# HazyResearch/flash-fft-conv

Measured on AMD Instinct MI355X. Metric: FFT-conv fwd+bwd seq/s, B=16 H=768 L=16384 fft=32768 bf16, higher is better.
Workload: dtype bf16; 1 GPU; FlashFFTConv(32768) B=16 H=768 L=16384 bf16, fwd+bwd incl. k->k_f and dk (BASELINE configs[1]); heads_per_rank=768, parallelism=head-shard x1 (no collective)

## Files before the change

flash-fft-conv_amd/csrc/ffc_body.h:

```cpp
#pragma once
#include <stdint.h>

#include "ffc_layout.h"
#include "ffc_plan.h"

#ifndef FFC_FN
#define FFC_FN inline __attribute__((always_inline))
#endif

namespace ffc {

struct ConvArgs {
  const void* u;
  const void* pregate;
  const void* postgate;
  void* y;
  const void* kf;
  const uint8_t* tab;
  PlanTabs t;
  int B, H, L;
  int npair;
  int nchunk, ppc;
  int conj_kf;
  int fast;
  float s_inv;
  float s_fwd;
  int flags;
  int stream;
  int persist;
  int R;
  int64_t sbu, sbg, sbp, sby;
  void* zsave;
  void* yraw;
  int sparse;
  unsigned long long* prof;
  const void* aux_in;
  void* aux_out;
  int64_t sbai, sbao;
  const float* kfuse_k;
  const void* kfuse_x;
  int kfuse_Lk, kfuse_fast;
  float kfuse_scale;
  const void* addend;
  int64_t sba;
};

struct Pass {
  int k0 = 0, R = 1;
  const uint8_t* mat_fwd = nullptr;
  const uint8_t* mat_inv = nullptr;
};

template <class B, class GEO, int DT>
struct Body {
  using f32 = typename B::f32;
  using i32 = typename B::i32;
  using u32 = typename B::u32;
  using pred = typename B::pred;
  using U2 = typename B::U2;
  using U4 = typename B::U4;
  using A16 = typename B::A16;
  using W4 = typename B::W4;

  struct Mat { W4 w[2][3]; };
  struct CT16 { A16 re, im; };
  struct Op { W4 r[2], i[2]; };

  static FFC_FN void load_mat(Mat& m, const uint8_t* p, i32 lane) {
#pragma unroll
// ... 1570 lines not shown
    }
  }
  static FFC_FN void z_load(const void* zs, int tau, KfRegs& z, bool nt = false) {
    const i32 lane = B::opaque(B::lane());
    const i32 c = lane & 31, hi = lane >> 5;
    if (nt) {
#pragma unroll
      for (int rq = 0; rq < 4; rq++) z.v[rq] = B::g_r128_nt(zs, ((hi + (tau * 8 + 2 * rq)) * 32 + c));
      return;
    }
#pragma unroll
    for (int rq = 0; rq < 4; rq++) z.v[rq] = B::g_r128(zs, ((hi + (tau * 8 + 2 * rq)) * 32 + c));
  }
  static FFC_FN uint8_t* z_slot(void* base, int h, int npair, int p) {
    return (uint8_t*)base + ((int64_t)h * npair + p) * ((int64_t)GEO::N * 4);
  }
  static FFC_FN uint8_t* z_slot_small(void* base, int h, int npair, int q, int R, int k0) {
    const int ntile = (npair + GEO::G - 1) / GEO::G;
    return (uint8_t*)base + (((int64_t)h * ntile + q) * R + k0) * 4096;
  }
  static FFC_FN uint8_t* z_slot_rp(void* base, int h, int npair, int p, int R, int k0) {
    return (uint8_t*)base + (((int64_t)h * npair + p) * R + k0) * ((int64_t)GEO::N * 4);
  }
  static FFC_FN void load_kf(const ConvArgs& a, int h, int tau, KfRegs& k) {
    const i32 lane = B::opaque(B::lane());
    const i32 c = lane & 31, hi = lane >> 5;
    const uint8_t* kfh = (const uint8_t*)a.kf + (int64_t)h * (GEO::NT * 1024 * 4);
    if (a.flags & 2) {
#pragma unroll
      for (int rq = 0; rq < 4; rq++) k.v[rq] = B::g_r128_nt(kfh, ((hi + (tau * 8 + 2 * rq)) * 32 + c));
      return;
    }
#pragma unroll
    for (int rq = 0; rq < 4; rq++) k.v[rq] = B::g_r128(kfh, ((hi + (tau * 8 + 2 * rq)) * 32 + c));
  }
  template <bool IP = false, bool SZ = false>
  static FFC_FN void inner_tile(const ConvArgs& a, int tau, const InnerRegs& R, Unit un, const KfRegs& kf, const InnerPass* ip = nullptr,
                                uint8_t* zs = nullptr) {
    A16 re, im;
    tile_fwd<true, IP>(tau, R, un, re, im, ip);
    if constexpr (SZ) {
      if (GEO::OUTER || zs) z_store(zs, 0, re, im, Z_STREAM);
    }
#pragma unroll
    for (int rq = 0; rq < 4; rq++) {
      u32 wv[4] = {kf.v[rq].x, kf.v[rq].y, kf.v[rq].z, kf.v[rq].w};
#pragma unroll
      for (int q = 0; q < 4; q++) {
        f32 kr = B::template unpack_lo<DT>(wv[q]), ki = B::template unpack_hi<DT>(wv[q]);
        if (a.conj_kf) ki = B::fconst(0.f) - ki;
// ... 726 lines not shown
```

flash-fft-conv_amd/csrc/ffc_k_bwd.hip:

```cpp
#include "ffc_bwd_launch.h"

template <int DT>
__global__ __launch_bounds__(256) void mul_rows_kernel(const uint16_t* __restrict__ x, const uint16_t* __restrict__ y, uint16_t* __restrict__ out,
                                                       int64_t HL, int64_t sbx, int64_t sby, int64_t sbo, int fast) {
  const int b = blockIdx.y;
  const uint16_t* xb = x + b * sbx; const uint16_t* yb = y + b * sby; uint16_t* ob = out + b * sbo;
  if (fast) {
    for (int64_t i = (int64_t)blockIdx.x * blockDim.x + threadIdx.x; i < HL / 8; i += (int64_t)gridDim.x * blockDim.x) {
      const u32x4v a = __builtin_nontemporal_load((const u32x4v*)xb + i), c = __builtin_nontemporal_load((const u32x4v*)yb + i);
      u32x4v o;
#pragma unroll
      for (int q = 0; q < 4; q++)
        o[q] = DevB::pack<DT>(DevB::unpack_lo<DT>(a[q]) * DevB::unpack_lo<DT>(c[q]), DevB::unpack_hi<DT>(a[q]) * DevB::unpack_hi<DT>(c[q]));
      __builtin_nontemporal_store(o, (u32x4v*)ob + i);
    }
  } else {
    for (int64_t i = (int64_t)blockIdx.x * blockDim.x + threadIdx.x; i < HL; i += (int64_t)gridDim.x * blockDim.x)
      ob[i] = (uint16_t)DevB::pack<DT>(DevB::unpack_lo<DT>(xb[i]) * DevB::unpack_lo<DT>(yb[i]), 0.f);
  }
}


extern "C" int ffc_conv_bwd(const ffc_plan* p, const void* dout, const void* u, const void* kf, const void* pregate,
                            const void* postgate, void* du, void* dpre, void* ws, int64_t B, int64_t H, int64_t L, void* stream) {
  return ffc_conv_bwd_gated(p, dout, u, kf, pregate, postgate, du, dpre, nullptr, ws, B, H, L, stream);
}
struct BwdCall {
  const void *dout, *u, *kf, *pregate, *postgate;
  void *du, *dpre, *dpost, *ws;
  int64_t B, H, L;
  void* stream;
  int64_t sb_dout, sb_u, sb_pre, sb_post, sb_du, sb_dpre, sb_dpost;
  const void *zin, *yraw;
  float* dk; int64_t Lk;
  void* dk_pair; float dk_pair_scale;
  bool* dk_done;
};
static BwdCall bwd_call(const void* dout, const void* u, const void* kf, const void* pregate, const void* postgate, void* du, void* dpre,
                        void* dpost, void* ws, int64_t B, int64_t H, int64_t L, void* stream) {
  BwdCall c{};
  c.dout = dout; c.u = u; c.kf = kf; c.pregate = pregate; c.postgate = postgate; c.du = du; c.dpre = dpre; c.dpost = dpost; c.ws = ws;
  c.B = B; c.H = H; c.L = L; c.stream = stream;
  return c;
}
static void bwd_strides(BwdCall* c, int64_t sb_dout, int64_t sb_u, int64_t sb_pre, int64_t sb_post, int64_t sb_du, int64_t sb_dpre, int64_t sb_dpost) {
  c->sb_dout = sb_dout; c->sb_u = sb_u; c->sb_pre = sb_pre; c->sb_post = sb_post; c->sb_du = sb_du; c->sb_dpre = sb_dpre; c->sb_dpost = sb_dpost;
}
static int conv_bwd_impl(const ffc_plan* p, const BwdCall& c) {
  const void *dout = c.dout, *u = c.u, *kf = c.kf, *pregate = c.pregate, *postgate = c.postgate, *zin = c.zin, *yraw = c.yraw;
  void *du = c.du, *dpre = c.dpre, *dpost = c.dpost, *ws = c.ws, *stream = c.stream;
  const int64_t B = c.B, H = c.H, L = c.L, Lk = c.Lk;
  int64_t sb_dout = c.sb_dout, sb_u = c.sb_u, sb_pre = c.sb_pre, sb_post = c.sb_post, sb_du = c.sb_du, sb_dpre = c.sb_dpre, sb_dpost = c.sb_dpost;
  if (!p || !dout || !kf || !du || !ws) return ffc_fail("null arg");
  if (!u && (!zin || pregate || postgate || dpre || (dpost && !yraw))) return ffc_fail("null u: only with saved spectra and no gates");
  if (yraw && !dpost) return ffc_fail("y_raw needs a dpost output");
  if (yraw && !zin && p->hp.N1 > 1) return ffc_fail("y_raw without the saved spectra: single-tile sizes (fft <= 2048) only");
  if (zin && (ffc_spectrum_bytes(p, B, H) == 0 || ((uintptr_t)zin & 15))) return ffc_fail("spectrum buffer: unsupported plan or misaligned");
  if (B <= 0 || H <= 0) return ffc_fail("empty batch/heads");
  if (L <= 0 || L > p->hp.N) return ffc_fail("L must be in (0, fft_size]");
// ... 27 lines not shown
  if (c.dk_pair && c.dk_done && !((uintptr_t)c.dk_pair & 15) && bwd_dk_form(p->hp, a.nchunk, p->env_flags, true) != DK_SEPARATE) {
    set_dk_tail(&d, nullptr, c.dk_pair, p->hp.N, c.dk_pair_scale, 1, p->d_blob_bf, p->hp_bf.tabs);
    *c.dk_done = true;
  }
  d.dpost = (p->hp.N1 > 1 || yraw) ? dpost : nullptr;
  d.zin = zin;
  d.yraw = yraw;
  if (yraw && p->hp.R > 1 && p->hp.N1 > 1) {
    const int64_t HL = H * L;
    const int fast = (HL % 8 == 0) && !((sb_dout | sb_dpost) & 7) && !(((uintptr_t)dout | (uintptr_t)yraw | (uintptr_t)dpost) & 15);
    int64_t nb = (HL / (fast ? 8 : 1) + 255) / 256;
    if (nb > 8192) nb = 8192;
    const dim3 grid((unsigned)nb, (unsigned)B), block(256);
    if (p->hp.dtype == DT_BF16)
      hipLaunchKernelGGL(mul_rows_kernel<DT_BF16>, grid, block, 0, (hipStream_t)stream, (const uint16_t*)dout, (const uint16_t*)yraw,
                         (uint16_t*)dpost, HL, sb_dout, HL, sb_dpost, fast);
    else
      hipLaunchKernelGGL(mul_rows_kernel<DT_F16>, grid, block, 0, (hipStream_t)stream, (const uint16_t*)dout, (const uint16_t*)yraw,
                         (uint16_t*)dpost, HL, sb_dout, HL, sb_dpost, fast);
    HIPCHK(hipGetLastError());
    d.dpost = nullptr; d.yraw = nullptr; dpost = nullptr;
  }
  if (d.dpost && ((((uintptr_t)dpost) | (uintptr_t)yraw) & 15)) a.fast = 0;
  int rc = (zin && p->hp.N1 > 1) ? ffc_bwdz_launch(p->hp.N, p->hp.dtype, d, (hipStream_t)stream)
                                 : ffc_dispatch<BwdLaunchZ<0>::T>(p->hp.N, p->hp.dtype, d, (hipStream_t)stream);
  if (rc || !dpost || d.dpost) return rc;
  return ffc_conv_fwd_strided(p, u, kf, pregate, dout, dpost, B, H, L, 0, sb_u, sb_pre, sb_dout, sb_dpost, stream);
}
extern "C" int ffc_conv_bwd_gated_strided(const ffc_plan* p, const void* dout, const void* u, const void* kf, const void* pregate,
                                          const void* postgate, void* du, void* dpre, void* dpost, void* ws, int64_t B, int64_t H,
                                          int64_t L, int64_t sb_dout, int64_t sb_u, int64_t sb_pre, int64_t sb_post,
                                          int64_t sb_du, int64_t sb_dpre, int64_t sb_dpost, void* stream) {
  BwdCall c = bwd_call(dout, u, kf, pregate, postgate, du, dpre, dpost, ws, B, H, L, stream);
  bwd_strides(&c, sb_dout, sb_u, sb_pre, sb_post, sb_du, sb_dpre, sb_dpost);
  return conv_bwd_impl(p, c);
}
extern "C" int ffc_conv_bwd_z(const ffc_plan* p, const void* dout, const void* u, const void* kf, const void* pregate,
                              const void* postgate, void* du, void* dpre, void* dpost, void* ws, const void* zin, int64_t B, int64_t H,
                              int64_t L, int64_t sb_dout, int64_t sb_u, int64_t sb_pre, int64_t sb_post,
                              int64_t sb_du, int64_t sb_dpre, int64_t sb_dpost, void* stream) {
  if (!zin) return ffc_fail("null spectrum buffer");
  BwdCall c = bwd_call(dout, u, kf, pregate, postgate, du, dpre, dpost, ws, B, H, L, stream);
  bwd_strides(&c, sb_dout, sb_u, sb_pre, sb_post, sb_du, sb_dpre, sb_dpost);
  c.zin = zin;
  return conv_bwd_impl(p, c);
}
// ... 1 lines not shown
                               const void* postgate, void* du, void* dpre, void* dpost, void* ws, const void* zin, const void* y_raw,
                               int64_t B, int64_t H, int64_t L, int64_t sb_dout, int64_t sb_u, int64_t sb_pre, int64_t sb_post,
                               int64_t sb_du, int64_t sb_dpre, int64_t sb_dpost, void* stream) {
  if ((!zin && !(p && p->hp.N1 <= 1)) || !y_raw || !dpost) return ffc_fail("null spectrum / y_raw / dpost buffer (y_raw alone: single-tile sizes, fft <= 2048)");
  BwdCall c = bwd_call(dout, u, kf, pregate, postgate, du, dpre, dpost, ws, B, H, L, stream);
  bwd_strides(&c, sb_dout, sb_u, sb_pre, sb_post, sb_du, sb_dpre, sb_dpost);
  c.zin = zin; c.yraw = y_raw;
  return conv_bwd_impl(p, c);
}
extern "C" int ffc_conv_bwd_gated(const ffc_plan* p, const void* dout, const void* u, const void* kf, const void* pregate,
                                  const void* postgate, void* du, void* dpre, void* dpost, void* ws, int64_t B, int64_t H,
                                  int64_t L, void* stream) {
  return ffc_conv_bwd_gated_strided(p, dout, u, kf, pregate, postgate, du, dpre, dpost, ws, B, H, L, 0, 0, 0, 0, 0, 0, 0, stream);
}

extern "C" int ffc_conv_bwd_k(const ffc_plan* p, const void* dout, const void* u, const void* kf, const void* pregate, const void* postgate,
                              void* du, void* dpre, void* dpost, void* ws, const void* zin, const void* y_raw, float* dk, int64_t Lk,
                              int64_t B, int64_t H, int64_t L, void* stream) {
  if (!dk) return ffc_fail("null dk");
  bool dk_done = false;
  BwdCall c = bwd_call(dout, u, kf, pregate, postgate, du, dpre, dpost, ws, B, H, L, stream);
  c.zin = zin; c.yraw = ((zin || p->hp.N1 <= 1) && y_raw && dpost) ? y_raw : nullptr;
  c.dk = dk; c.Lk = Lk; c.dk_done = &dk_done;
  int rc = conv_bwd_impl(p, c);
  if (rc || dk_done) return rc;
  return ffc_kernel_ifft_grad(p, ws, B, H, Lk, dk, stream);
}

extern "C" int ffc_conv_bwd_kx(const ffc_plan* p, const void* dout, const void* u, const void* kf, void* du, void* ws, const void* zin,
                               void* outpair, float scale, int64_t B, int64_t H, int64_t L, void* stream) {
  if (!outpair) return ffc_fail("null outpair");
  bool dk_done = false;
  BwdCall c = bwd_call(dout, u, kf, nullptr, nullptr, du, nullptr, nullptr, ws, B, H, L, stream);
  c.zin = zin; c.dk_pair = outpair; c.dk_pair_scale = scale; c.dk_done = &dk_done;
  int rc = conv_bwd_impl(p, c);
  if (rc || dk_done) return rc;
  return ffc_kernel_ifft_grad_c(p, ws, B, H, outpair, scale, stream);
}
```

flash-fft-conv_amd/csrc/ffc_modes.h:

```cpp
#pragma once
#include "ffc_body.h"

namespace ffc {

struct KfArgs {
  const float* k;
  void* kf;
  const uint8_t* tab;
  PlanTabs t;
  int H, Lk;
  float scale;
  float s_fwd;
  float prescale;
  const void* xpair;
  int fast;
  int R;
};

struct DkfArgs {
  ConvArgs c;
  const void* dout;
  float* ws;
  int64_t sbd, sbdu, sbdpre, sbdpost;
  void* du;
// ... 175 lines not shown
#pragma unroll
      for (int q = 0; q < 4; q++) w[q] = B::template pack<DT>(re[4 * rq + q] * a.scale, im[4 * rq + q] * a.scale);
      v.x = w[0]; v.y = w[1]; v.z = w[2]; v.w = w[3];
      if constexpr (GEO::OUTER) {
        pred ok = (c * 0 + unit_id) < a.H * hmul;
        i32 idx = ((hi + (tau * 8 + 2 * rq)) * 32 + c) + unit_id * (GEO::NT * 256);
        B::g_w128(a.kf, idx, v, ok);
      } else {
        i32 V = hi * 4 + 8 * rq;
        i32 sV = V / GEO::N3, k3 = V % GEO::N3, sU = c / GEO::N2, k2 = c % GEO::N2;
        i32 hd = sU * GEO::SV + sV + unit_id * GEO::G;
        pred ok = hd < a.H;
#pragma unroll
        for (int su = 0; su < GEO::SU; su++)
#pragma unroll
          for (int sv = 0; sv < GEO::SV; sv++) {
            i32 rho = (k3 + sv * GEO::N3) >> 2;
            i32 idx = (rho * 32 + (k2 + su * GEO::N2)) + hd * 256;
            B::g_w128(a.kf, idx, v, ok);
          }
      }
    }
  }
  static FFC_FN void kf_store_flat(const KfArgs& a, int hrow, const A16& re, const A16& im, int hlim) {
    const i32 lane = B::opaque(B::lane());
    const i32 c = lane & 31, hi = lane >> 5;
#pragma unroll
    for (int rq = 0; rq < 4; rq++) {
      U4 v;
      v.x = B::template pack<DT>(re[4 * rq] * a.scale, im[4 * rq] * a.scale);
      v.y = B::template pack<DT>(re[4 * rq + 1] * a.scale, im[4 * rq + 1] * a.scale);
      v.z = B::template pack<DT>(re[4 * rq + 2] * a.scale, im[4 * rq + 2] * a.scale);
      v.w = B::template pack<DT>(re[4 * rq + 3] * a.scale, im[4 * rq + 3] * a.scale);
      B::g_w128(a.kf, ((hi + 2 * rq) * 32 + c) + hrow * 256, v, (c * 0 + hrow) < hlim);
    }
  }
  static FFC_FN void kfft(const KfArgs& a, int wg) {
    BD::setup_tables(a.tab, a.t);
    const int wv = B::wave();
    Unit un;
    un.wq = wv % GEO::NW;
    const int u = wv / GEO::NW;
    un.eb = u * GEO::EBYTES;
    const int unit_id = wg * GEO::UPW + u;
    const int nunits = GEO::OUTER ? a.H : (a.H + GEO::G - 1) / GEO::G;
    const bool act = unit_id < nunits;
// ... 24 lines not shown
              kf_store(a, unit_id * a.R + k0, un.wq * GEO::TPW + tt, re, im, a.R);
            }
          }
          B::barrier();
        }
        return;
      }
    }
    if constexpr (GEO::OUTER) {
      if (act) {
        if (a.xpair) {
          ConvArgs cv{};
          cv.u = a.xpair; cv.B = 2; cv.H = a.H; cv.L = GEO::N; cv.fast = 1; cv.sbu = (int64_t)a.H * GEO::N;
          BD::rows_in(cv, unit_id, 0, un);
        } else {
          k_rows_in(a, unit_id, un);
        }
        B::lds_fence();
        if ((GEO::N1 / 2) * GEO::Mi >= a.Lk) BD::template outer_stage<true, true>(a.Lk, un, a.s_fwd);
        else BD::template outer_stage<true, false>(a.Lk, un, a.s_fwd);
      }
      B::barrier();
      if (act) {
#pragma unroll 1
        for (int tt = 0; tt < GEO::TPW; tt++) {
          A16 re, im;
          BD::tile_fwd(un.wq * GEO::TPW + tt, R, un, re, im);
          kf_store(a, unit_id, un.wq * GEO::TPW + tt, re, im);
        }
      }
    } else if (a.R > 1) {
      if constexpr (GEO::N == 1024) {
        BD::setup_tables_ipass(a.tab, a.t, a.R);
        if (act) {
#pragma unroll 1
          for (int k0 = 0; k0 < a.R; k0++) {
            Pass ps; ps.k0 = k0; ps.R = a.R;
            InnerPass ip;
            BD::load_inner_pass(ip, k0);
            k_rows_in_rp(a, unit_id, un, ps);
            B::lds_fence();
            A16 re, im;
            BD::template tile_fwd<true, true, false, true>(0, R, un, re, im, &ip);
            kf_store_flat(a, unit_id * a.R + k0, re, im, a.H * a.R);
            B::lds_fence();
          }
        }
      }
    } else {
      if (act) {
        k_rows_in(a, unit_id, un);
// ... 12 lines not shown
    a.k = c.kfuse_k; a.kf = const_cast<void*>(c.kf); a.H = c.H; a.Lk = c.kfuse_Lk; a.scale = c.kfuse_scale; a.s_fwd = c.s_fwd;
    a.prescale = DT == DT_F16 ? 256.f : 1.f;
    a.fast = c.kfuse_fast;
    Unit un;
    un.wq = B::wave() % GEO::NW;
    un.eb = 0;
    if (unit == 0) {
      if (c.kfuse_x) {
        ConvArgs cv{};
        cv.u = c.kfuse_x; cv.B = 2; cv.H = c.H; cv.L = GEO::N; cv.fast = 1; cv.sbu = (int64_t)c.H * GEO::N;
        BD::rows_in(cv, h, 0, un);
        a.Lk = GEO::N; a.prescale = 1.0f;
      } else {
        k_rows_in(a, h, un);
      }
      B::lds_fence();
      if ((GEO::N1 / 2) * GEO::Mi >= a.Lk) BD::template outer_stage<true, true>(a.Lk, un, a.s_fwd);
      else BD::template outer_stage<true, false>(a.Lk, un, a.s_fwd);
    }
    B::barrier();
    if (unit == 0) {
      InnerRegs R;
      BD::load_inner(R, un);
#pragma unroll 1
      for (int tt = 0; tt < GEO::TPW; tt++) {
        A16 re, im;
        BD::tile_fwd(un.wq * GEO::TPW + tt, R, un, re, im);
        kf_store(a, h, un.wq * GEO::TPW + tt, re, im);
      }
    }
    B::barrier();
  }

  struct ZReg { u32 r[8], i[8]; };
  static FFC_FN void z_pack(const A16& re, const A16& im, ZReg& z) {
#pragma unroll
    for (int q = 0; q < 8; q++) {
      z.r[q] = B::template pack<DT>(re[2 * q], re[2 * q + 1]);
      z.i[q] = B::template pack<DT>(im[2 * q], im[2 * q + 1]);
    }
  }
  using BD::z_store;
  using BD::z_load;
  static FFC_FN void w_accum_z(float* slab, int tau, bool first, const typename BD::KfRegs& zv, const A16& re, const A16& im) {
    const i32 lane = B::opaque(B::lane());
    const i32 c = lane & 31, hi = lane >> 5;
#pragma unroll
    for (int rq = 0; rq < 4; rq++) {
      i32 idx = ((hi + (tau * 8 + 2 * rq)) * 32 + c) * 2;
      u32 wv[4] = {zv.v[rq].x, zv.v[rq].y, zv.v[rq].z, zv.v[rq].w};
      f32 wr[4], wi[4];
// ... 248 lines not shown
        }
        re[r] = sr * d.dk_scale; im[r] = si * d.dk_scale;
      }
      BD::template tile_inv<false>(d.c.s_inv, un.wq * GEO::TPW + T, R, un, re, im);
    }
    B::barrier();
  }
  static FFC_FN void dk_tail_multi(const DkfArgs& d, int h, int u, int wq) {
    static_assert(GEO::UPW > 1 && GEO::TPW == 4, "dk tail: sums in registers");
    const Unit un = unit_of(u, wq);
    const i32 lane = B::opaque(B::lane());
    B::barrier();
    InnerRegs R;
    if (u == 0) BD::template load_inner<false>(R, un);
    dk_tail_tile_multi<0>(d, u, un, R, lane); dk_tail_tile_multi<1>(d, u, un, R, lane);
    dk_tail_tile_multi<2>(d, u, un, R, lane); dk_tail_tile_multi<3>(d, u, un, R, lane);
    if (u == 0) {
      BD::template outer_stage<false, false>(d.Lk, un);
      B::lds_fence();
      dk_tail_rows(d, h, un);
    }
    B::barrier();
  }
  template <bool WITH_DX, bool RP = false, bool ZSAVED = false>
  static FFC_FN void bwd_tiles(const ConvArgs& a, int h, Unit un, const InnerRegs& R, const void* zs, float* slab, bool first, WAcc& W,
                               Pass ps = Pass(), bool z_stream = false, bool second = false) {
    static_assert(GEO::TPW == 4, "one accumulator block a[32 T ..] per tile slot of the wave");
    constexpr bool FOLD = BD::CAN_FOLD && GEO::N1 == 32 && WITH_DX && !RP && ZSAVED;
    const uint8_t* fold = FOLD ? a.tab + a.t.fold : nullptr;
    typename BD::KfRegs zv;
    typename BD::Mat2 fa;
    if constexpr (FOLD) BD::load_mat2_issue(fa, fold + (un.wq * GEO::TPW) * 6144, B::opaque(B::lane()));
#pragma unroll 1
    for (int tt = 0; tt < GEO::TPW; tt++) {
      const int tau = un.wq * GEO::TPW + tt;
      if constexpr (WITH_DX && GEO::NW > 1) {
        if (tt == GEO::TPW / 2) { if (second) B::template setprio<2>(); else B::template setprio<1>(); }
      }
      z_load(zs, tau, zv, z_stream || (a.flags & 4) != 0);
      typename BD::KfRegs kf;
      constexpr bool KFL = FOLD;
      if constexpr (WITH_DX && !KFL) BD::load_kf(a, h, tau, kf);
      A16 re, im;
      BD::template tile_fwd<false, false, FOLD>(tau, R, un, re, im, nullptr, fold, FOLD ? &fa : nullptr);
      if constexpr (WITH_DX && KFL) BD::load_kf(a, h, tau, kf);
      switch (tt) {
        case 0: w_acc_tile<0>(zv, re, im); break;
        case 1: w_acc_tile<1>(zv, re, im); break;
        case 2: w_acc_tile<2>(zv, re, im); break;
        default: w_acc_tile<3>(zv, re, im); break;
      }
      if constexpr (WITH_DX) {
        typename BD::Mat2 g[2];
        if constexpr (FOLD) {
          const i32 lane = B::opaque(B::lane());
          BD::load_mat2_issue(g[0], fold + (2 * GEO::NT + tau) * 6144, lane);
          BD::load_mat2_issue(g[1], fold + (3 * GEO::NT + tau) * 6144, lane);
        }
        kf_conj_mul(kf, re, im);
        if constexpr (FOLD) {
          const int tn = tt + 1 < GEO::TPW ? tau + 1 : tau;
          BD::load_mat2_issue(fa, fold + tn * 6144, B::opaque(B::lane()));
        }
        BD::template tile_inv<false, RP, false, FOLD>(a.s_inv, tau, R, un, re, im, 0, ps, nullptr, fold, FOLD ? g : nullptr);
      }
    }
  }
  template <bool HALF = false, bool RP = false>
  static FFC_FN void dkf(const DkfArgs& d, int h, int chunk, int wg_linear, int k0 = 0, int wv_in = 0) {
    const ConvArgs& a = d.c;
    const Pass ps = RP ? make_pass(a.tab, a.t, a.R, k0) : Pass();
    constexpr int NCX = HALF ? BD::NCH / 2 : BD::NCH;
    if constexpr (!RP) BD::setup_tables(a.tab, a.t);
    const int wv = RP ? wv_in : B::wave();
    Unit un;
    un.wq = wv % GEO::NW;
    const int u = wv / GEO::NW;
    un.eb = u * GEO::EBYTES;
    const int p0 = chunk * a.ppc;
    int p1 = p0 + a.ppc;
    if (p1 > a.npair) p1 = a.npair;
    ConvArgs av = a;
// ... 116 lines not shown
#pragma unroll
    for (int rq = 0; rq < 4; rq++) {
      u32 wv[4] = {z.v[rq].x, z.v[rq].y, z.v[rq].z, z.v[rq].w};
#pragma unroll
      for (int q = 0; q < 4; q++) {
        re[4 * rq + q] = B::template unpack_lo<DT>(wv[q]);
        im[4 * rq + q] = B::template unpack_hi<DT>(wv[q]);
      }
    }
  }
  static FFC_FN void kf_plain_mul(const typename BD::KfRegs& kf, A16& re, A16& im) {
    typename BD::CT16 k;
#pragma unroll
    for (int rq = 0; rq < 4; rq++) {
      u32 wv[4] = {kf.v[rq].x, kf.v[rq].y, kf.v[rq].z, kf.v[rq].w};
#pragma unroll
      for (int q = 0; q < 4; q++) {
        k.re[4 * rq + q] = B::template unpack_lo<DT>(wv[q]);
        k.im[4 * rq + q] = B::template unpack_hi<DT>(wv[q]);
      }
    }
    BD::cmul(re, im, k);
  }
  static FFC_FN void kf_conj_mul(const typename BD::KfRegs& kf, A16& re, A16& im) {
    typename BD::CT16 k;
#pragma unroll
    for (int rq = 0; rq < 4; rq++) {
      u32 wv[4] = {kf.v[rq].x, kf.v[rq].y, kf.v[rq].z, kf.v[rq].w};
#pragma unroll
      for (int q = 0; q < 4; q++) {
        k.re[4 * rq + q] = B::template unpack_lo<DT>(wv[q]);
        k.im[4 * rq + q] = B::template unpack_hi<DT>(wv[q]);
      }
    }
    BD::cmul_conj(re, im, k);
  }
  template <bool HALF = false, bool RP = false, bool SETUP = true, int ZM = -1, bool GS = false, bool PL = false>
  static FFC_FN void bwd(const DkfArgs& d, int h, int chunk, int wg_linear, int k0 = 0, int wv_in = 0) {
    static_assert(!GS || (HALF && !RP && BD::HALF_C), "direct-store phase C: single-pass fft 32768, L <= N/2");
    static_assert(!PL || (GS && ZM >= 0), "plain input rows: a form of the direct-store kernels");
    const ConvArgs& a = d.c;
    const Pass ps = RP ? make_pass(a.tab, a.t, a.R, k0) : Pass();
    const int hk = RP ? h * a.R + k0 : h;
    constexpr int NCX = HALF ? BD::NCH / 2 : BD::NCH;
    if constexpr (!RP && SETUP) BD::setup_tables(a.tab, a.t);
    const int wv = RP ? wv_in : B::wave();
    Unit un;
    un.wq = wv % GEO::NW;
    const int u = wv / GEO::NW;
    un.eb = u * GEO::EBYTES;
    const int p0 = chunk * a.ppc;
    int p1 = p0 + a.ppc;
    if (p1 > a.npair) p1 = a.npair;
    ConvArgs av = a;
    ConvArgs ad = a;
    ad.u = d.dout; ad.pregate = a.postgate; ad.sbu = d.sbd; ad.sbg = a.sbp;
    ConvArgs ao = a;
// ... 109 lines not shown
          }
          BD::unit_barrier();
          FFC_BPRIO(1)
          if (dpost_tf) {
            if (act) {
              BD::template outer_stage<false, HALF, RP>(a.L, un, 1.0f, ps, a.flags);
              B::lds_fence();
              if constexpr (RP) BD::template rows_out_rp<NCX>(aq, h, p, un, ps);
              else BD::template rows_out<NCX>(aq, h, p, un);
            }
          }
          if (act) {
            if constexpr (RP) BD::template rows_in_rp<NCX>(ad, h, p, un, ps);
            else BD::template rows_in_sel<NCX, PL>(ad, h, p, un);
            B::lds_fence();
            FFC_BPRIO(0)
            BD::template outer_stage<true, HALF, RP>(a.L, un, a.s_fwd, ps);
          }
        }
        BD::unit_barrier();
        FFC_BPRIO(3)
        if (act) {
          BD::template load_inner<false>(R, un);
          bwd_tiles<true, RP, ZM == 1>(a, hk, un, R, zp, slab, it == 0, W, ps, have_z && BD::Z_STREAM, second);
        } else if (it == 0) {
#pragma unroll 1
          for (int tt = GEO::TPW; tt < GEO::TPW; tt++) w_zero(slab, un.wq * GEO::TPW + tt);
        }
        BD::unit_barrier();
        FFC_BPRIO(3)
        if constexpr (GS) {
          if (act) {
            BD::template outer_inv_half<true, ROT>(un, &ao, h, p, [&]() {
              if constexpr (DMA_OK) {
                if (dma && p + GEO::UPW < p1) { B::lds_wait0(); BD::rows_dma(ad, h, p + GEO::UPW, un); }
              }
            });
          }
          if constexpr (ROT) {
            if (p + GEO::UPW < p1) {
              FFC_BPRIO(1)
              BD::template rows_dma_finish<BD::HALF_C_STORES>(ad, p + GEO::UPW, un);
            }
          }
        } else if (act) {
          BD::template outer_stage<false, HALF, RP>(a.L, un, 1.0f, ps, a.flags);
          B::lds_fence();
// ... 399 lines not shown
```

flash-fft-conv_amd/csrc/ffc_route.h:

```cpp
#pragma once
#include <stdint.h>
#include <type_traits>
#include "ffc_body.h"
#include "ffc_modes.h"
#include "ffc_big.h"

namespace ffc {

template <class F>
inline int pick(F&& f) { return f(); }
template <class F, class... Bs>
inline int pick(F&& f, bool b, Bs... bs) {
  return b ? pick([&](auto... r) { return f(std::true_type{}, r...); }, bs...)
           : pick([&](auto... r) { return f(std::false_type{}, r...); }, bs...);
}
template <class F>
inline int level_dispatch(int n0, bool f16, bool fwd, F&& f) {
  return pick([&](auto n32, auto h, auto fw) -> int {
    return f(std::integral_constant<int, decltype(n32)::value ? 32 : 16>{}, std::integral_constant<int, decltype(h)::value ? DT_F16 : DT_BF16>{}, fw);
  }, n0 == 32, f16, fwd);
}

template <class F>
inline bool with_geo(int N, F&& f) {
// ... 90 lines not shown
  r.lds_max = r.lds = GEO::LDS_BYTES;
  if (c.R > 1 && GEO::OUTER) {
    if (GEO::N != 32768) { r.err = NO_MULTI_PASS; return r; }
    r.multi_pass = true;
    r.half = 16 * GEO::Mi >= c.L;
    r.fastk = !dkf && c.fast && (FFC_RP_FASTK != 0);
    return r;
  }
  if (GEO::OUTER) {
    if (GEO::NW == 1 && c.persist > 0 && r.grid > c.persist) r.grid = c.persist;
    r.half = (GEO::N1 / 2) * GEO::Mi >= c.L;
    r.gs = !dkf && direct_store_ok<GEO>(r.half, false, c.fast, !c.pregate && !d.dpre, c.flags);
    r.pl = plain_rows_ok(r.gs, !c.postgate && !d.dpost && !d.yraw && !(c.flags & 8), c.flags);
    return r;
  }
  r.small = true;
  if (c.R > 1 && GEO::N != 1024) { r.err = NO_MULTI_PASS; return r; }
  r.lds_max = GEO::LDS_BYTES + 2 * IPASS_BYTES;
  r.lds = GEO::LDS_BYTES + (c.R > 1 ? c.R * IPASS_BYTES : 0);
  if (!dkf) r.grid = cap_two_per_cu(r.grid, c.persist);
  return r;
}

inline bool fwd_takes_kfft(const HostPlan& hp, int nchunk, int sparse, int flags) {
  return nchunk == 1 && hp.N >= 8192 && hp.N <= 32768 && hp.R == 1 && !sparse && !(flags & 64);
}
enum { DK_SEPARATE = 0, DK_TAIL = 1, DK_TAIL_MULTI = 2 };
inline bool bwd_takes_dk(const HostPlan& hp, int nchunk, int flags) {
  return nchunk == 1 && hp.N >= ((flags & 128) ? 8192 : 16384) && hp.N <= 32768 && hp.R == 1 && !(flags & 32);
}
inline bool bwd_takes_dk_multi(const HostPlan& hp, int nchunk, int flags) {
  return nchunk == 1 && hp.R > 1 && hp.N1 > 1 && hp.dtype == DT_BF16 && !(flags & 32);
}
inline int bwd_dk_form(const HostPlan& hp, int nchunk, int flags, bool complex_rows) {
  if (bwd_takes_dk(hp, nchunk, flags)) return DK_TAIL;
  return (!complex_rows && bwd_takes_dk_multi(hp, nchunk, flags)) ? DK_TAIL_MULTI : DK_SEPARATE;
}
inline void set_dk_tail(DkfArgs* d, float* dk, void* pair, int Lk, float scale, int fast, const uint8_t* tab_bf, const PlanTabs& t_bf) {
  d->dk_out = dk; d->dk_pair = pair; d->Lk = Lk; d->dk_scale = scale; d->dk_fast = fast;
  d->tab_bf = tab_bf; d->t_bf = t_bf;
}

inline int decode_dtype(int dtype, int dir, BigArgs* a) {
  a->lf32 = (dtype & 16) ? 1 : 0;
  a->half = (dtype & 32) ? 1 : 0;
  const int e = (dtype >> 8) & 0xff;
// ... 38 lines not shown
```

flash-fft-conv_amd/csrc/ffc_sim.cpp:

```cpp
#include <math.h>
#include <pthread.h>
#include <stdint.h>
#include <stdlib.h>
#include <string.h>

#include <atomic>
#include <thread>
#include <vector>

#define FFC_FN inline __attribute__((always_inline))
#include "ffc_body.h"
#include "ffc_modes.h"
#include "ffc_big.h"
#include "ffc_route.h"

namespace ffc {

template <class T>
struct Vec {
  T v[64];
  Vec() {}
  Vec(T s) { for (int i = 0; i < 64; i++) v[i] = s; }
};
#define VOP(op)                                                                           \
// ... 7 lines not shown
#undef VOP
template <class T> inline Vec<T> operator<<(const Vec<T>& a, int s) { Vec<T> r; for (int i = 0; i < 64; i++) r.v[i] = a.v[i] << s; return r; }
template <class T> inline Vec<T> operator>>(const Vec<T>& a, int s) { Vec<T> r; for (int i = 0; i < 64; i++) r.v[i] = a.v[i] >> s; return r; }
inline Vec<uint32_t> operator&(const Vec<uint32_t>& a, unsigned b) { Vec<uint32_t> r; for (int i = 0; i < 64; i++) r.v[i] = a.v[i] & b; return r; }
inline Vec<int> operator*(const Vec<int>& a, long b) { return a * (int)b; }
inline Vec<bool> operator<(const Vec<int>& a, int b) { Vec<bool> r; for (int i = 0; i < 64; i++) r.v[i] = a.v[i] < b; return r; }
inline Vec<bool> operator<(const Vec<int>& a, const Vec<int>& b) { Vec<bool> r; for (int i = 0; i < 64; i++) r.v[i] = a.v[i] < b.v[i]; return r; }
inline Vec<bool> operator>=(const Vec<int>& a, int b) { Vec<bool> r; for (int i = 0; i < 64; i++) r.v[i] = a.v[i] >= b; return r; }
inline Vec<bool> operator&&(const Vec<bool>& a, const Vec<bool>& b) { Vec<bool> r; for (int i = 0; i < 64; i++) r.v[i] = a.v[i] && b.v[i]; return r; }
inline Vec<bool> operator&&(const Vec<bool>& a, bool b) { Vec<bool> r; for (int i = 0; i < 64; i++) r.v[i] = a.v[i] && b; return r; }

struct WgCtx {
  std::vector<uint8_t> lds;
  pthread_barrier_t bar;
  int nwaves;
};
static thread_local WgCtx* g_wg = nullptr;
static thread_local int g_wave = 0;
static thread_local Vec<float> g_agpr[128];
static std::atomic<long> g_dma_count{0};
static std::atomic<long> g_gs_count{0};
static std::atomic<long> g_pl_count{0};
static int g_sim_flags = 0;

static inline float dt_to_f32(int DT, uint16_t h) { return DT == DT_BF16 ? bf16_to_f32(h) : f16_to_f32(h); }
static inline uint16_t f32_to_dt(int DT, float f) { return DT == DT_BF16 ? f32_to_bf16(f) : f32_to_f16(f); }

struct SimB {
  static constexpr bool LEAN_OUTER = false;
  static constexpr bool FAST_ONLY = false;
  static constexpr bool HAS_ADD = false;
  using f32 = Vec<float>;
  using i32 = Vec<int>;
  using u32 = Vec<uint32_t>;
  using pred = Vec<bool>;
  struct U2 { u32 x, y; };
  struct U4 { u32 x, y, z, w; };
  struct A16 { f32 v[16]; f32& operator[](int i) { return v[i]; } const f32& operator[](int i) const { return v[i]; } };
  struct W4 { u32 v[4]; u32& operator[](int i) { return v[i]; } const u32& operator[](int i) const { return v[i]; } };
  struct A4 { f32 v[4]; f32& operator[](int i) { return v[i]; } const f32& operator[](int i) const { return v[i]; } };
  static A4 a4_zero() { A4 z; for (int i = 0; i < 4; i++) z.v[i] = f32(0.f); return z; }
  template <bool CONJ> static void cmul16(A16& re, A16& im, const A16& tr, const A16& ti) {
    for (int r = 0; r < 16; r++) {
      f32 a = re[r], b = im[r];
      if (!CONJ) { re[r] = a * tr[r] - b * ti[r]; im[r] = a * ti[r] + b * tr[r]; }
      else { re[r] = a * tr[r] + b * ti[r]; im[r] = b * tr[r] - a * ti[r]; }
// ... 324 lines not shown
  }, r.multi_pass, r.half, r.sz, r.sp);
}

template <template <class, int> class FN, class... A>
static int dispatch(int N, int dtype, A&&... args) {
  int rc = 0;
  const bool found = with_geo(N, [&](auto geo) {
    using GEO = decltype(geo);
    rc = dtype == DT_BF16 ? FN<GEO, DT_BF16>::run(args...) : FN<GEO, DT_F16>::run(args...);
  });
  return found ? rc : -1;
}
template <class GEO, int DT> struct ConvRun { static int run(const ConvArgs& a) { return sim_conv_t<GEO, DT>(a); } };
template <class GEO, int DT> struct ConvResRun { static int run(const ConvArgs& a) { return sim_conv_t<GEO, DT, SimBA>(a); } };
template <class GEO, int DT> struct KfRun {
  static int run(const KfArgs& a) {
    const int nunits = GEO::OUTER ? a.H : (a.H + GEO::G - 1) / GEO::G;
    for (int wg = 0; wg < (nunits + GEO::UPW - 1) / GEO::UPW; wg++)
      run_wg(GEO::WGW, sim_lds<GEO>(), [&]() { Modes<SimB, GEO, DT>::kfft(a, wg); });
    return 0;
  }
};
template <class GEO, int DT, bool DKF>
static int sim_bwd_t(const DkfArgs& d) {
  using MO = Modes<SimBO, GEO, DT>;
  const BwdRoute r = bwd_route<GEO>(d, DKF);
  if (r.err) return NO_KERNEL;
  const int H = d.c.H, nchunk = d.c.nchunk, lds = sim_lds<GEO>();
  if (r.gs) {
    if constexpr (GEO::N == 32768) {
      g_gs_count++;
      if (r.pl) g_pl_count++;
      return pick([&](auto zm, auto pl) -> int {
        return sim_jobs(H, nchunk, lds, [&](int h, int c) {
          MO::template bwd<true, false, true, decltype(zm)::value ? 1 : 0, true, decltype(pl)::value>(d, h, c, h * nchunk + c);
        });
      }, d.zin != nullptr, r.pl);
    } else {
      return NO_KERNEL;
    }
  }
  return pick([&](auto mp, auto half, auto fastk, auto zm) -> int {
    constexpr bool MP = decltype(mp)::value, HALF = decltype(half)::value, FASTK = decltype(fastk)::value, ZM = decltype(zm)::value;
    if constexpr (!GEO::OUTER) {
      if constexpr (MP || HALF || FASTK || ZM) return NO_KERNEL;
      else if constexpr (DKF) return sim_jobs(H, nchunk, lds, [&](int h, int c) { MO::dkf(d, h, c, h * nchunk + c); });
      else return sim_jobs(H, nchunk, lds, [&](int h, int c) { MO::bwd(d, h, c, h * nchunk + c); });
    } else if constexpr (MP) {
      if constexpr (GEO::N != 32768 || (DKF && (FASTK || ZM))) {
        return NO_KERNEL;
// ... 103 lines not shown
int ffcsim_outer_inv_half(int dtype, const uint16_t* e_in, uint16_t* e_out) {
  HostPlan p;
  if (!build_plan(32768, dtype, &p)) return -1;
  if (dtype == DT_BF16) sim_outer_inv_half<DT_BF16>(p, e_in, e_out);
  else sim_outer_inv_half<DT_F16>(p, e_in, e_out);
  return 0;
}

int ffcsim_plan_info(int N, int dtype, int* nt, double* s_fwd, double* s_k, int32_t* kf_freq ) {
  HostPlan p;
  if (!build_plan(N, dtype, &p)) return -1;
  *nt = p.NT * p.R; *s_fwd = p.s_fwd; *s_k = p.s_k;
  if (kf_freq) memcpy(kf_freq, p.kf_freq.data(), p.kf_freq.size() * 4);
  return 0;
}

static int g_sparse_rows = 0;
void ffcsim_set_sparse(int rows) { g_sparse_rows = rows; }
static void* g_z = nullptr; static void* g_yraw = nullptr; static int g_flags = 0;
void ffcsim_set_z(void* z, void* yraw, int flags) { g_z = z; g_yraw = yraw; g_flags = flags; }
long ffcsim_dma_count() { return g_dma_count.exchange(0); }
long ffcsim_gs_count() { return g_gs_count.exchange(0); }
long ffcsim_pl_count() { return g_pl_count.exchange(0); }
void ffcsim_set_flags(int flags) { g_sim_flags = flags; }
static float* g_dk_out = nullptr; static int g_dk_lk = 0;
void ffcsim_set_fused_dk(float* dk, int Lk) { g_dk_out = dk; g_dk_lk = Lk; }
static const float* g_kfuse_k = nullptr; static int g_kfuse_lk = 0;
void ffcsim_set_fused_k(const float* k, int Lk) { g_kfuse_k = k; g_kfuse_lk = Lk; }
static const void* g_kfuse_x = nullptr; static float g_kfuse_xscale = 1.f;
void ffcsim_set_fused_kx(const void* xpair, float scale) { g_kfuse_x = xpair; g_kfuse_xscale = scale; }
static void* g_dk_pair = nullptr; static float g_dk_pair_scale = 1.f;
void ffcsim_set_fused_dkpair(void* outpair, float scale) { g_dk_pair = outpair; g_dk_pair_scale = scale; }
static int g_big_pipe = 0;
void ffcsim_set_big_pipe(int on) { g_big_pipe = on; }
int ffcsim_conv_fwd(int N, int dtype, const void* u, const void* kf, const void* pregate, const void* postgate,
                    void* y, int B, int H, int L, int conj_kf) {
  HostPlan p;
  if (!build_plan(N, dtype, &p)) return -1;
  if (L > N || L <= 0) return -2;
  ConvArgs a{};
  a.u = u; a.pregate = pregate; a.postgate = postgate; a.y = y; a.kf = kf;
  a.tab = p.blob.data(); a.t = p.tabs;
  a.B = B; a.H = H; a.L = L; a.npair = (B + 1) / 2;
  a.sbu = a.sbg = a.sbp = a.sby = (int64_t)H * L;
  a.nchunk = 1; a.ppc = a.npair; a.conj_kf = conj_kf; a.s_inv = (float)p.s_inv; a.s_fwd = (float)p.s_fwd;
  a.fast = (L % 8 == 0) && !g_force_slow;
// ... 311 lines not shown
```

Before: 11.49 million seq/s.

## Exploit Hermitian symmetry of real-kernel spectrum in k_f build and bwd reads

The kernel FFT for fft 32768 now computes only the lower half of the tiles and writes each tile together with its conjugate-mirrored counterpart, using the Hermitian symmetry of a real kernel's spectrum. In the pipelined backward pass, the second pass can read the mirrored k_f tile (lane-reversed, element-reversed, imaginary part negated) instead of the direct one, presumably to improve cache locality or reuse between the paired passes. This is gated on a new KF_MIRROR flag that is set only when the kernel is real and the pipelined route is used. It adds lane permutation and select work, plus correctness risk at the Nyquist and DC tiles.

```diff
diff --git a/flash-fft-conv_amd/csrc/ffc_body.h b/flash-fft-conv_amd/csrc/ffc_body.h
--- a/flash-fft-conv_amd/csrc/ffc_body.h
+++ b/flash-fft-conv_amd/csrc/ffc_body.h
@@ -45,6 +45,10 @@
   int64_t sba;
 };
 
+enum {
+  KF_MIRROR = 1 << 16,
+};
+
 struct Pass {
   int k0 = 0, R = 1;
   const uint8_t* mat_fwd = nullptr;
@@ -1661,10 +1665,28 @@
   static FFC_FN uint8_t* z_slot_rp(void* base, int h, int npair, int p, int R, int k0) {
     return (uint8_t*)base + (((int64_t)h * npair + p) * R + k0) * ((int64_t)GEO::N * 4);
   }
-  static FFC_FN void load_kf(const ConvArgs& a, int h, int tau, KfRegs& k) {
+  template <bool MIR = false>
+  static FFC_FN void load_kf(const ConvArgs& a, int h, int tau, KfRegs& k, bool mir = false) {
     const i32 lane = B::opaque(B::lane());
     const i32 c = lane & 31, hi = lane >> 5;
     const uint8_t* kfh = (const uint8_t*)a.kf + (int64_t)h * (GEO::NT * 1024 * 4);
+    if constexpr (MIR) {
+      static_assert(GEO::N == 32768, "mirrored k_f reads: the tile digits of fft 32768");
+      if (!(a.flags & 2)) {
+        const int ts = mir ? GEO::NT - tau : tau;
+        const i32 l0 = lane ^ (mir ? 63 : 0);
+        const pred m = (lane * 0 + (mir ? 1 : 0)) >= 1;
+        KfRegs t;
+#pragma unroll
+        for (int j = 0; j < 4; j++) t.v[j] = B::g_r128(kfh, l0 + (ts * 8 + 2 * j) * 32);
+#pragma unroll
+        for (int rq = 0; rq < 4; rq++) {
+          k.v[rq].x = B::sel(m, t.v[3 - rq].w, t.v[rq].x); k.v[rq].y = B::sel(m, t.v[3 - rq].z, t.v[rq].y);
+          k.v[rq].z = B::sel(m, t.v[3 - rq].y, t.v[rq].z); k.v[rq].w = B::sel(m, t.v[3 - rq].x, t.v[rq].w);
+        }
+        return;
+      }
+    }
     if (a.flags & 2) {
 #pragma unroll
       for (int rq = 0; rq < 4; rq++) k.v[rq] = B::g_r128_nt(kfh, ((hi + (tau * 8 + 2 * rq)) * 32 + c));
diff --git a/flash-fft-conv_amd/csrc/ffc_k_bwd.hip b/flash-fft-conv_amd/csrc/ffc_k_bwd.hip
--- a/flash-fft-conv_amd/csrc/ffc_k_bwd.hip
+++ b/flash-fft-conv_amd/csrc/ffc_k_bwd.hip
@@ -35,6 +35,7 @@
   float* dk; int64_t Lk;
   void* dk_pair; float dk_pair_scale;
   bool* dk_done;
+  bool kf_real;
 };
 static BwdCall bwd_call(const void* dout, const void* u, const void* kf, const void* pregate, const void* postgate, void* du, void* dpre,
                         void* dpost, void* ws, int64_t B, int64_t H, int64_t L, void* stream) {
@@ -108,6 +109,7 @@
     d.dpost = nullptr; d.yraw = nullptr; dpost = nullptr;
   }
   if (d.dpost && ((((uintptr_t)dpost) | (uintptr_t)yraw) & 15)) a.fast = 0;
+  if (p->hp.N == 32768 && p->hp.R == 1) a.flags |= kf_mirror_flags(c.kf_real, bwd_route<Geo<32, 32, 32>>(d, false).pl, a.flags);
   int rc = (zin && p->hp.N1 > 1) ? ffc_bwdz_launch(p->hp.N, p->hp.dtype, d, (hipStream_t)stream)
                                  : ffc_dispatch<BwdLaunchZ<0>::T>(p->hp.N, p->hp.dtype, d, (hipStream_t)stream);
   if (rc || !dpost || d.dpost) return rc;
@@ -155,6 +157,7 @@
   BwdCall c = bwd_call(dout, u, kf, pregate, postgate, du, dpre, dpost, ws, B, H, L, stream);
   c.zin = zin; c.yraw = ((zin || p->hp.N1 <= 1) && y_raw && dpost) ? y_raw : nullptr;
   c.dk = dk; c.Lk = Lk; c.dk_done = &dk_done;
+  c.kf_real = true;
   int rc = conv_bwd_impl(p, c);
   if (rc || dk_done) return rc;
   return ffc_kernel_ifft_grad(p, ws, B, H, Lk, dk, stream);
diff --git a/flash-fft-conv_amd/csrc/ffc_modes.h b/flash-fft-conv_amd/csrc/ffc_modes.h
--- a/flash-fft-conv_amd/csrc/ffc_modes.h
+++ b/flash-fft-conv_amd/csrc/ffc_modes.h
@@ -221,6 +221,35 @@
       }
     }
   }
+  static FFC_FN void kf_store_herm(const KfArgs& a, int unit_id, int tau, const A16& re, const A16& im) {
+    static_assert(GEO::N == 32768, "Hermitian k_f store: the tile digits of fft 32768");
+    const i32 lane = B::opaque(B::lane());
+    const pred ok = (lane * 0 + unit_id) < a.H;
+    const pred okm = ok && (tau != 0);
+#pragma unroll
+    for (int rq = 0; rq < 4; rq++) {
+      u32 w[4];
+#pragma unroll
+      for (int q = 0; q < 4; q++) w[q] = B::template pack<DT>(re[4 * rq + q] * a.scale, im[4 * rq + q] * a.scale);
+      U4 v, m;
+      v.x = w[0]; v.y = w[1]; v.z = w[2]; v.w = w[3];
+      const u32 sg = B::uconst(0x80000000u);
+      m.x = w[3] ^ sg; m.y = w[2] ^ sg; m.z = w[1] ^ sg; m.w = w[0] ^ sg;
+      const bool lower = tau != GEO::NT / 2 || rq < 2;
+      const i32 idx = (lane + (tau * 8 + 2 * rq) * 32) + unit_id * (GEO::NT * 256);
+      const i32 idm = ((lane ^ 63) + ((GEO::NT - tau) * 8 + 2 * (3 - rq)) * 32) + unit_id * (GEO::NT * 256);
+      B::g_w128(a.kf, idx, v, ok && lower);
+      B::g_w128(a.kf, tau ? idm : idx, m, okm && lower);
+    }
+  }
+  static FFC_FN void kf_tiles_herm(const KfArgs& a, int unit_id, Unit un, const InnerRegs& R) {
+#pragma unroll 1
+    for (int tau = un.wq; tau <= GEO::NT / 2; tau += GEO::NW) {
+      A16 re, im;
+      BD::tile_fwd(tau, R, un, re, im);
+      kf_store_herm(a, unit_id, tau, re, im);
+    }
+  }
   static FFC_FN void kf_store_flat(const KfArgs& a, int hrow, const A16& re, const A16& im, int hlim) {
     const i32 lane = B::opaque(B::lane());
     const i32 c = lane & 31, hi = lane >> 5;
@@ -291,11 +320,17 @@
       }
       B::barrier();
       if (act) {
-#pragma unroll 1
-        for (int tt = 0; tt < GEO::TPW; tt++) {
-          A16 re, im;
-          BD::tile_fwd(un.wq * GEO::TPW + tt, R, un, re, im);
-          kf_store(a, unit_id, un.wq * GEO::TPW + tt, re, im);
+        bool herm = false;
+        if constexpr (GEO::N == 32768) herm = !a.xpair;
+        if (herm) {
+          if constexpr (GEO::N == 32768) kf_tiles_herm(a, unit_id, un, R);
+        } else {
+#pragma unroll 1
+          for (int tt = 0; tt < GEO::TPW; tt++) {
+            A16 re, im;
+            BD::tile_fwd(un.wq * GEO::TPW + tt, R, un, re, im);
+            kf_store(a, unit_id, un.wq * GEO::TPW + tt, re, im);
+          }
         }
       }
     } else if (a.R > 1) {
@@ -354,11 +389,17 @@
     if (unit == 0) {
       InnerRegs R;
       BD::load_inner(R, un);
-#pragma unroll 1
-      for (int tt = 0; tt < GEO::TPW; tt++) {
-        A16 re, im;
-        BD::tile_fwd(un.wq * GEO::TPW + tt, R, un, re, im);
-        kf_store(a, h, un.wq * GEO::TPW + tt, re, im);
+      bool herm = false;
+      if constexpr (GEO::N == 32768) herm = !c.kfuse_x;
+      if (herm) {
+        if constexpr (GEO::N == 32768) kf_tiles_herm(a, h, un, R);
+      } else {
+#pragma unroll 1
+        for (int tt = 0; tt < GEO::TPW; tt++) {
+          A16 re, im;
+          BD::tile_fwd(un.wq * GEO::TPW + tt, R, un, re, im);
+          kf_store(a, h, un.wq * GEO::TPW + tt, re, im);
+        }
       }
     }
     B::barrier();
@@ -653,7 +694,7 @@
     }
     B::barrier();
   }
-  template <bool WITH_DX, bool RP = false, bool ZSAVED = false>
+  template <bool WITH_DX, bool RP = false, bool ZSAVED = false, bool MIR = false>
   static FFC_FN void bwd_tiles(const ConvArgs& a, int h, Unit un, const InnerRegs& R, const void* zs, float* slab, bool first, WAcc& W,
                                Pass ps = Pass(), bool z_stream = false, bool second = false) {
     static_assert(GEO::TPW == 4, "one accumulator block a[32 T ..] per tile slot of the wave");
@@ -662,6 +703,8 @@
     typename BD::KfRegs zv;
     typename BD::Mat2 fa;
     if constexpr (FOLD) BD::load_mat2_issue(fa, fold + (un.wq * GEO::TPW) * 6144, B::opaque(B::lane()));
+    static_assert(!MIR || (WITH_DX && !RP && GEO::N == 32768), "mirrored k_f reads: single-pass fft 32768");
+    const bool mir = MIR && second && (a.flags & KF_MIRROR) != 0;
 #pragma unroll 1
     for (int tt = 0; tt < GEO::TPW; tt++) {
       const int tau = un.wq * GEO::TPW + tt;
@@ -671,10 +714,10 @@
       z_load(zs, tau, zv, z_stream || (a.flags & 4) != 0);
       typename BD::KfRegs kf;
       constexpr bool KFL = FOLD;
-      if constexpr (WITH_DX && !KFL) BD::load_kf(a, h, tau, kf);
+      if constexpr (WITH_DX && !KFL) BD::template load_kf<MIR>(a, h, tau, kf, mir);
       A16 re, im;
       BD::template tile_fwd<false, false, FOLD>(tau, R, un, re, im, nullptr, fold, FOLD ? &fa : nullptr);
-      if constexpr (WITH_DX && KFL) BD::load_kf(a, h, tau, kf);
+      if constexpr (WITH_DX && KFL) BD::template load_kf<MIR>(a, h, tau, kf, mir);
       switch (tt) {
         case 0: w_acc_tile<0>(zv, re, im); break;
         case 1: w_acc_tile<1>(zv, re, im); break;
@@ -688,7 +731,7 @@
           BD::load_mat2_issue(g[0], fold + (2 * GEO::NT + tau) * 6144, lane);
           BD::load_mat2_issue(g[1], fold + (3 * GEO::NT + tau) * 6144, lane);
         }
-        kf_conj_mul(kf, re, im);
+        kf_conj_mul<MIR>(kf, re, im, mir);
         if constexpr (FOLD) {
           const int tn = tt + 1 < GEO::TPW ? tau + 1 : tau;
           BD::load_mat2_issue(fa, fold + tn * 6144, B::opaque(B::lane()));
@@ -851,7 +894,8 @@
     }
     BD::cmul(re, im, k);
   }
-  static FFC_FN void kf_conj_mul(const typename BD::KfRegs& kf, A16& re, A16& im) {
+  template <bool MIR = false>
+  static FFC_FN void kf_conj_mul(const typename BD::KfRegs& kf, A16& re, A16& im, bool mir = false) {
     typename BD::CT16 k;
 #pragma unroll
     for (int rq = 0; rq < 4; rq++) {
@@ -862,6 +906,7 @@
         k.im[4 * rq + q] = B::template unpack_hi<DT>(wv[q]);
       }
     }
+    if constexpr (MIR) k.im = B::a16_scale(k.im, mir ? -1.0f : 1.0f);
     BD::cmul_conj(re, im, k);
   }
   template <bool HALF = false, bool RP = false, bool SETUP = true, int ZM = -1, bool GS = false, bool PL = false>
@@ -1017,7 +1062,7 @@
         FFC_BPRIO(3)
         if (act) {
           BD::template load_inner<false>(R, un);
-          bwd_tiles<true, RP, ZM == 1>(a, hk, un, R, zp, slab, it == 0, W, ps, have_z && BD::Z_STREAM, second);
+          bwd_tiles<true, RP, ZM == 1, PL && !RP && GEO::N == 32768>(a, hk, un, R, zp, slab, it == 0, W, ps, have_z && BD::Z_STREAM, second);
         } else if (it == 0) {
 #pragma unroll 1
           for (int tt = GEO::TPW; tt < GEO::TPW; tt++) w_zero(slab, un.wq * GEO::TPW + tt);
diff --git a/flash-fft-conv_amd/csrc/ffc_route.h b/flash-fft-conv_amd/csrc/ffc_route.h
--- a/flash-fft-conv_amd/csrc/ffc_route.h
+++ b/flash-fft-conv_amd/csrc/ffc_route.h
@@ -136,6 +136,11 @@
   return r;
 }
 
+inline int kf_mirror_flags(bool kf_real, bool pl, int flags) {
+  if (!kf_real || !pl || (flags & (1024 | 2))) return 0;
+  return KF_MIRROR;
+}
+
 inline bool fwd_takes_kfft(const HostPlan& hp, int nchunk, int sparse, int flags) {
   return nchunk == 1 && hp.N >= 8192 && hp.N <= 32768 && hp.R == 1 && !sparse && !(flags & 64);
 }
diff --git a/flash-fft-conv_amd/csrc/ffc_sim.cpp b/flash-fft-conv_amd/csrc/ffc_sim.cpp
--- a/flash-fft-conv_amd/csrc/ffc_sim.cpp
+++ b/flash-fft-conv_amd/csrc/ffc_sim.cpp
@@ -53,6 +53,8 @@
 static std::atomic<long> g_gs_count{0};
 static std::atomic<long> g_pl_count{0};
 static int g_sim_flags = 0;
+static std::atomic<long> g_kfm_count{0};
+static bool g_kf_real = false;
 
 static inline float dt_to_f32(int DT, uint16_t h) { return DT == DT_BF16 ? bf16_to_f32(h) : f16_to_f32(h); }
 static inline uint16_t f32_to_dt(int DT, float f) { return DT == DT_BF16 ? f32_to_bf16(f) : f32_to_f16(f); }
@@ -423,10 +425,13 @@
   }
 };
 template <class GEO, int DT, bool DKF>
-static int sim_bwd_t(const DkfArgs& d) {
+static int sim_bwd_t(const DkfArgs& d_in) {
   using MO = Modes<SimBO, GEO, DT>;
+  DkfArgs d = d_in;
   const BwdRoute r = bwd_route<GEO>(d, DKF);
   if (r.err) return NO_KERNEL;
+  if (GEO::N == 32768 && d.c.R <= 1 && !DKF) d.c.flags |= kf_mirror_flags(g_kf_real, r.pl, d.c.flags);
+  if (d.c.flags & KF_MIRROR) g_kfm_count++;
   const int H = d.c.H, nchunk = d.c.nchunk, lds = sim_lds<GEO>();
   if (r.gs) {
     if constexpr (GEO::N == 32768) {
@@ -576,6 +581,8 @@
 long ffcsim_dma_count() { return g_dma_count.exchange(0); }
 long ffcsim_gs_count() { return g_gs_count.exchange(0); }
 long ffcsim_pl_count() { return g_pl_count.exchange(0); }
+long ffcsim_kf_mirror_count() { return g_kfm_count.exchange(0); }
+void ffcsim_set_kf_real(int on) { g_kf_real = on != 0; }
 void ffcsim_set_flags(int flags) { g_sim_flags = flags; }
 static float* g_dk_out = nullptr; static int g_dk_lk = 0;
 void ffcsim_set_fused_dk(float* dk, int Lk) { g_dk_out = dk; g_dk_lk = Lk; }
```

Result: no change. 11.42 million seq/s (-0.7%).
